# philip-bl/dctn

Measured on AMD Instinct MI355X. Metric: EPS-contraction windows/sec (fwd+bwd), higher is better.
Workload: dtype bf16; 1 GPU; cfg2 EPS[(3,4)]+linear bf16 B1024/GPU; parallelism=dp1

## Files before the change

dctn_amd/_lib.py:

```python
from __future__ import annotations

import ctypes
import os
import subprocess
from typing import Optional, Sequence

import torch

_HERE = os.path.dirname(os.path.abspath(__file__))
LIB_PATH = os.path.join(_HERE, "libdctn_amd.so")
CSRC = os.path.join(_HERE, "csrc")

F32, F64, BF16 = 0, 1, 2
PREC_EXACT, PREC_BF16, PREC_SPLIT, PREC_MASK = 0, 1, 2, 0xFF
OPT_F32_PREFER_HALVES, OPT_SMALL_CHUNKS, OPT_MAIN_KERNEL_ONLY, OPT_GENERIC_KERNELS = 1 << 8, 1 << 9, 1 << 10, 1 << 11
OPT_HEAD_FEATURES_BLOCKED4 = 1 << 12
ERR_BAD_SHAPE, ERR_BAD_DTYPE, ERR_UNSUPPORTED, ERR_WORKSPACE, ERR_LAUNCH, ERR_NULL = -1, -2, -3, -4, -5, -6
SAVED, PARTIAL = 1, 2
(EPS_FAMILY_GENERIC, EPS_FAMILY_Q2REG, EPS_FAMILY_BIGCORE_F32, EPS_FAMILY_HALVES, EPS_FAMILY_Q2REG_F32,
 EPS_FAMILY_BIGCORE_BF16X3) = range(6)
SBS_MATRIX_CORE_SWEEP = 1 << 8
SBS_WIDE_SWEEP = 1 << 9
BATCH_SRC_U8_TABLE, BATCH_SRC_ROWS = 0, 1
BATCH_IDENTITY_ORDER, BATCH_PAD_TAIL = 1, 2
# ... 16 lines not shown
    "dctn_device_limits": (c_int, [_IntP, _IntP]),
    "dctn_eps_family": (c_int, [c_int] * 9),
    "dctn_eps_fwd_workspace_bytes": (c_size, [c_int] * 7 + [c_int] * 2),
    "dctn_eps_fwd": (c_int, [c_void, _I64x5, c_void, c_void, c_void, c_size] + [c_int] * 7 + [c_int, c_int, c_void]),
    "dctn_eps_saved_bytes": (c_size, [c_int] * 7 + [c_int] * 2),
    "dctn_eps_fwd_save": (c_int, [c_void, _I64x5, c_void, c_void, c_void, c_size, c_void, c_size] + [c_int] * 7 + [c_int, c_int, c_void]),
    "dctn_eps_bwd_saved": (c_int, [c_void, _I64x5, c_void, c_void, c_void, c_size, c_void, c_void, c_void, c_size]
                           + [c_int] * 7 + [c_int, c_int, c_void]),
    "dctn_eps_fwd_stats_workspace_bytes": (c_size, [c_int] * 7 + [c_int] * 2),
    "dctn_eps_fwd_stats": (c_int, [c_void, _I64x5, c_void, c_void, c_void, c_size] + [c_int] * 7 + [c_int, c_int, c_void]),
    "dctn_eps_bwd_workspace_bytes": (c_size, [c_int] * 7 + [c_int] * 4),
    "dctn_eps_bwd": (c_int, [c_void, _I64x5, c_void, c_void, c_void, c_void, c_void, c_size]
                     + [c_int] * 7 + [c_int, c_int, c_void]),
    "dctn_eps_head_fwd": (c_int, [c_void, _I64x5, c_void, c_void, c_void, c_void, c_void] + [c_int] * 8 + [c_int, c_int, c_void]),
    "dctn_eps_head_bwd_workspace_bytes": (c_size, [c_int] * 8 + [c_int, c_int]),
    "dctn_eps_head_bwd": (c_int, [c_void, _I64x5, c_void, c_void, c_void, c_void, c_void, c_void, c_void, c_size]
                          + [c_int] * 8 + [c_int, c_int, c_void]),
    "dctn_ce_loss_fwd": (c_int, [c_void, c_void, c_void, c_i64, c_int, c_int, c_void]),
    "dctn_ce_loss_fwd_grad": (c_int, [c_void, c_void, c_void, c_void, c_i64, c_int, c_int, c_void]),
    "dctn_ce_loss_bwd": (c_int, [c_void, c_void, c_void, c_void, c_i64, c_int, c_int, c_void]),
    "dctn_sgd_l2_num_partials": (c_int, [c_i64]),
    "dctn_sgd_l2_step": (c_int, [c_void, c_void, c_void, c_void, c_i64, c_i64, ctypes.c_float, ctypes.c_float,
                                 ctypes.c_float, c_int, c_int, c_void]),
    "dctn_sgd_l2_step_master": (c_int, [c_void] * 5 + [c_i64, c_i64, ctypes.c_float, ctypes.c_float, ctypes.c_float,
                                        c_int, c_void]),
    "dctn_adam_state_bytes": (c_size, []),
    "dctn_adam_l2_num_partials": (c_int, [c_i64]),
    "dctn_adam_l2_step": (c_int, [c_void] * 6 + [c_i64, c_i64, ctypes.c_double, ctypes.c_double, ctypes.c_float,
                                  ctypes.c_float, ctypes.c_float, c_int, c_void]),
    "dctn_adam_l2_step_master": (c_int, [c_void] * 7 + [c_i64, c_i64, ctypes.c_double, ctypes.c_double, ctypes.c_float,
# ... 221 lines not shown
```

dctn_amd/csrc/capi.hip:

```cpp
#include "common.h"

#include <stdio.h>
#include <stdlib.h>

#include <algorithm>
#include <atomic>

static std::atomic<const char*> g_last_kernel{"none"};
void dctn_set_last_kernel(const char* name) { g_last_kernel.store(name, std::memory_order_relaxed); }

const DctnDev& dctn_dev() {
  static const DctnDev d = [] {
    DctnDev r{256, 160 * 1024};
    int dev = 0, v = 0;
    if (hipGetDevice(&dev) == hipSuccess) {
      if (hipDeviceGetAttribute(&v, hipDeviceAttributeMultiprocessorCount, dev) == hipSuccess && v > 0) r.cus = v;
      if (hipDeviceGetAttribute(&v, hipDeviceAttributeMaxSharedMemoryPerMultiprocessor, dev) == hipSuccess && v >= 64 * 1024) r.lds = v;
    }
    int cus = 0, lds = 0;
    const char* lim = getenv("DCTN_DEVICE_LIMITS");
    if (lim && sscanf(lim, "%d,%d", &cus, &lds) == 2) {
      if (cus > 0 && cus < r.cus) r.cus = cus;
      if (lds > 0 && lds < r.lds) r.lds = lds;
    }
// ... 144 lines not shown
                           int dtype, int policy) {
  if (!dtype_ok(dtype)) return DCTN_ERR_BAD_DTYPE;
  if (Cout < 1) return DCTN_ERR_BAD_SHAPE;
  const int blk = policy & DCTN_OPT_HEAD_FEATURES_BLOCKED4;
  const int rc = eps_fill_params(p, x_strides, C, B, H, W, Q, K, O, policy & ~blk);
  p.opts |= blk;
  return rc;
}

static bool eps_head_next(const EpsP& p, int rc) {
  return rc == DCTN_ERR_UNSUPPORTED && !(p.opts & DCTN_OPT_HEAD_FEATURES_BLOCKED4);
}

extern "C" {

int dctn_version(void) { return 507; }

const char* dctn_last_kernel(void) { return g_last_kernel.load(std::memory_order_relaxed); }

int dctn_device_limits(int* cus, int* lds_bytes) {
  if (!cus || !lds_bytes) return DCTN_ERR_NULL;
  *cus = dctn_dev().cus;
  *lds_bytes = dctn_dev().lds;
  return DCTN_OK;
}

const char* dctn_strerror(int code) {
  switch (code) {
    case DCTN_OK: return "ok";
    case DCTN_ERR_BAD_SHAPE: return "inconsistent shape";
    case DCTN_ERR_BAD_DTYPE: return "unknown dtype code";
// ... 119 lines not shown
  if (rc != DCTN_OK) return rc;
  const int precision = policy & DCTN_PREC_MASK;
  hipStream_t st = (hipStream_t)stream;
  rc = eps_head_fwd_mfma(x, core, head_weight, head_bias, features, logits, p, Cout, dtype, precision, st);
  if (!eps_head_next(p, rc)) return rc;
  return eps_head_fwd_q2f32(x, core, head_weight, head_bias, features, logits, p, Cout, dtype, precision, st);
}

size_t dctn_eps_head_bwd_workspace_bytes(int C, int B, int H, int W, int Q, int K, int O, int Cout, int dtype,
                                         int policy) {
  EpsP p;
  const int precision = policy & DCTN_PREC_MASK;
  if (!eps_query_params(p, C, B, H, W, Q, K, O, policy & ~DCTN_OPT_HEAD_FEATURES_BLOCKED4)) return 0;
  const size_t a = eps_head_bwd_mfma_workspace(p, Cout, dtype, precision), b = eps_head_bwd_q2f32_workspace(p, Cout, dtype, precision);
  return (a > b ? a : b) + 256;
}

int dctn_eps_head_bwd(const void* x, const int64_t x_strides[5], const void* features, const void* dLogits,
                      const void* head_weight, void* dCore, void* dWeight, void* dBias, void* workspace,
                      size_t workspace_bytes, int C, int B, int H, int W, int Q, int K, int O, int Cout,
                      int dtype, int policy, void* stream) {
  if (!x || !features || !dLogits || !head_weight || !dCore || !x_strides) return DCTN_ERR_NULL;
  EpsP p;
  int rc = eps_head_params(p, x_strides, C, B, H, W, Q, K, O, Cout, dtype, policy);
  if (rc != DCTN_OK) return rc;
  const int precision = policy & DCTN_PREC_MASK;
  hipStream_t st = (hipStream_t)stream;
  rc = eps_head_bwd_mfma(x, features, dLogits, head_weight, dCore, dWeight, dBias, workspace, workspace_bytes, p, Cout, dtype,
                         precision, st);
  if (!eps_head_next(p, rc)) return rc;
// ... 81 lines not shown
```

dctn_amd/csrc/common.h:

```cpp
#pragma once
#include <hip/hip_runtime.h>
#include <stdint.h>

#include "../../include/dctn_amd.h"

typedef __bf16 bf16_t;

template <typename S> struct AccOf { typedef float type; };
template <> struct AccOf<double> { typedef double type; };

#define DCTN_WAVE 64

#ifndef DCTN_WT_FEATURES
#define DCTN_WT_FEATURES 16
#endif
#ifndef DCTN_WT_TILES
#define DCTN_WT_TILES 0
#endif

struct DctnDev { int cus; int lds; };
const DctnDev& dctn_dev();
int dctn_lds_wg_max();
long long dctn_resident_wgs(size_t lds_bytes, int lo, int hi);
bool dctn_lds_optin(const void* fn, size_t bytes);
// ... 103 lines not shown
int eps_fwd_halves(const void* x, const void* core, void* out, void* ws, size_t ws_bytes, const EpsP& p, int dtype,
                   hipStream_t st, void* saved = nullptr);
size_t eps_bwd_halves_workspace(const EpsP& p, int dtype, int need_dx, int need_dcore);
int eps_bwd_halves(const void* x, const void* core, const void* dY, void* dX, void* dCore, void* ws, size_t ws_bytes,
                   const EpsP& p, int dtype, hipStream_t st, const void* saved = nullptr, size_t saved_bytes = 0);

int eps_fwd_mfma(const void* x, const void* core, void* out, const EpsP& p, int dtype,
                 int precision, hipStream_t st, double* stats = nullptr);
int eps_out_stats(const void* y, long long n, int dtype, double* stats, hipStream_t st);
size_t eps_bwd_mfma_workspace(const EpsP& p, int dtype, int precision, int need_dx, int need_dcore);
int eps_bwd_mfma(const void* x, const void* core, const void* dY, void* dX, void* dCore, void* ws,
                 size_t ws_bytes, const EpsP& p, int dtype, int precision, hipStream_t st);
int eps_head_fwd_mfma(const void* x, const void* core, const void* head_w, const void* bias, void* feat, void* logits,
                      const EpsP& p, int Cout, int dtype, int precision, hipStream_t st);
size_t eps_head_bwd_mfma_workspace(const EpsP& p, int Cout, int dtype, int precision);
int eps_head_bwd_mfma(const void* x, const void* feat, const void* dLogits, const void* head_w, void* dCore,
                      void* dW, void* dBias, void* ws, size_t ws_bytes, const EpsP& p, int Cout, int dtype,
                      int precision, hipStream_t st);

struct SbsShape {
  int n;
  const int *out_sizes, *bond_sizes, *pos_h, *pos_w;
  int C, B, H, W, q, dtype;
};
static inline SbsShape sbs_string(SbsShape many, int i) {
  many.out_sizes += i * many.n;
  many.bond_sizes += i * many.n;
  many.pos_h += i * many.n;
  many.pos_w += i * many.n;
  return many;
// ... 35 lines not shown
```

dctn_amd/csrc/eps_mfma.hip:

```cpp
#include "common.h"

#include <cstdlib>
#include <type_traits>

typedef __attribute__((ext_vector_type(8))) __bf16 bf16x8;
typedef __attribute__((ext_vector_type(16))) float f32x16;
typedef __attribute__((ext_vector_type(8))) float f32x8;
typedef __attribute__((ext_vector_type(2))) int int2v;
typedef __attribute__((ext_vector_type(4))) int int4v;
typedef __attribute__((ext_vector_type(2))) float f32x2;

namespace {

constexpr int ilog2(int v) { return v <= 1 ? 0 : 1 + ilog2(v >> 1); }

template <typename S> __device__ __forceinline__ float to_f32(S v) { return (float)v; }

__device__ __forceinline__ float half_sum(float v) {
  const int iv = __float_as_int(v);
  const int2v r = __builtin_amdgcn_permlane32_swap(iv, iv, false, false);
  return __int_as_float(r[0]) + __int_as_float(r[1]);
}

__device__ __forceinline__ void swap_halves(float& a, float& b) {
// ... 33 lines not shown
  const int g = lane >> 4, q = (lane >> 2) & 3, pp = lane & 3;
  const int lc = 2 * (g & 1) + (pp >> 1), half = pp & 1;
  const int row = 8 * (g >> 1) + q;
  t.rd_lo = row * LROW + (((lc + (row >> 1)) & 3) << 3) + 4 * half;
  t.rd_hi = (row + 4) * LROW + (((lc + ((row + 4) >> 1)) & 3) << 3) + 4 * half;
  return t;
}
__device__ __forceinline__ bf16x8 tr_frag(const short* tile, int ks, const TrLane& t) {
  typedef __attribute__((address_space(3))) s16x4 lds_s16x4;
  const s16x4 lo = __builtin_amdgcn_ds_read_tr16_b64_v4i16((lds_s16x4*)(tile + t.rd_lo + ks * 16 * LROW));
  const s16x4 hi = __builtin_amdgcn_ds_read_tr16_b64_v4i16((lds_s16x4*)(tile + t.rd_hi + ks * 16 * LROW));
  const s16x8 v = {lo[0], lo[1], lo[2], lo[3], hi[0], hi[1], hi[2], hi[3]};
  return __builtin_bit_cast(bf16x8, v);
}

struct FastDiv {
  unsigned M, s1, s2;
};
__device__ __forceinline__ unsigned fdiv(unsigned n, const FastDiv& d) {
  const unsigned t = __umulhi(d.M, n);
  return (t + ((n - t) >> d.s1)) >> d.s2;
}

#define MFMA_MAXN 16
struct MfmaP {
  int C, B, K, O, Ho, Wo;
  int P;
  int npg;
  int spc, nchunks;
  unsigned foffb[MFMA_MAXN];
  unsigned rowoffb[MFMA_MAXN];
  unsigned s1b, s2b, s3b, s4b;
  unsigned x_bytes;
  unsigned o_bytes, o_s1b;
  FastDiv div_wo;
  int rowvec_ok;
  int vec_ok;
  int Cout;
  unsigned hw_rowb, hw_bytes;
  int ncb;
  int skew;
  int opts;
#ifdef DCTN_STAMPS
  unsigned long long* stamps;
#endif
};

#ifdef DCTN_STAMPS
#define DCTN_STAMP(P, SLOT)                                                                      \
  do {                                                                                           \
    __builtin_amdgcn_sched_barrier(0);                                                           \
    unsigned long long t_;                                                                       \
    asm volatile("s_memrealtime %0\n\ts_waitcnt lgkmcnt(0)" : "=s"(t_)::"memory");               \
    if ((P).stamps && threadIdx.x == 0) (P).stamps[(long long)blockIdx.x * 8 + (SLOT)] = t_;     \
    __builtin_amdgcn_sched_barrier(0);                                                           \
  } while (0)
// ... 212 lines not shown
  } else {
#pragma unroll
    for (int o = 0; o < OP; ++o)
      if (o < O) {
        if constexpr (sizeof(S) == 2)
          __builtin_amdgcn_raw_buffer_store_b16((unsigned short)(pack_bf16(v[o], 0.f) & 0xffffu), rs, voff,
                                                soff + 2u * o, 0);
        else
          __builtin_amdgcn_raw_buffer_store_b32(__float_as_uint(v[o]), rs, voff, soff + 4u * o, 0);
      }
  }
}

struct WaveJob {
  int b0, b1;
  unsigned voff_x;
  unsigned voff_o;
  int pos;
  bool valid;
};
__device__ __forceinline__ WaveJob wave_job(const MfmaP& p, int waves_per_block, int esz, bool grouped = false) {
  const int nb = gridDim.x;
  const int vb = (nb % 8 == 0) ? (int)(blockIdx.x % 8) * (nb / 8) + (int)(blockIdx.x / 8) : (int)blockIdx.x;
  const int wave = __builtin_amdgcn_readfirstlane(vb * waves_per_block + (int)(threadIdx.x >> 6));
  int chunk = wave / p.npg, pg = wave - chunk * p.npg;
  if (grouped) {
    const int cb = vb / p.npg;
    pg = vb - cb * p.npg;
    chunk = __builtin_amdgcn_readfirstlane(cb * waves_per_block + (int)(threadIdx.x >> 6));
    if (cb >= p.ncb) chunk = p.nchunks;
  }
  WaveJob j;
  j.b0 = chunk < p.nchunks ? chunk * p.spc : 0;
  j.b1 = chunk < p.nchunks ? (j.b0 + p.spc < p.B ? j.b0 + p.spc : p.B) : 0;
  if (grouped && p.skew > 0) {
    const int w = __builtin_amdgcn_readfirstlane((int)(threadIdx.x >> 6)), half = waves_per_block / 2;
    const int n_old = p.spc + p.skew, n_young = p.spc - p.skew;
    const int s0 = (vb / p.npg) * waves_per_block * p.spc + (w < half ? w * n_old : half * n_old + (w - half) * n_young);
    const int s1 = s0 + (w < half ? n_old : n_young);
    const bool live = vb / p.npg < p.ncb && s0 < p.B;
    j.b0 = live ? s0 : 0;
    j.b1 = live ? (s1 < p.B ? s1 : p.B) : 0;
  }
  j.pos = pg * 64 + (int)(threadIdx.x & 63);
  j.valid = j.pos < p.P;
  const unsigned pu = j.valid ? (unsigned)j.pos : 0u;
  const unsigned ho = fdiv(pu, p.div_wo), wo = pu - ho * (unsigned)p.Wo;
  j.voff_x = j.valid ? ho * p.s2b + wo * p.s3b : p.x_bytes;
  j.voff_o = j.valid ? pu * (unsigned)(p.O * esz) : p.o_bytes;
  return j;
}

template <int N0>
__device__ __forceinline__ void build_p0(const float (*xv)[2], bf16x8 (&X)[(1 << N0) / 16],
                                         bf16x8 (&Y)[(1 << N0) / 16]) {
  constexpr int KS = (1 << N0) / 16;
  const f32x2 x1 = {xv[N0 - 1][0], xv[N0 - 1][1]}, x2 = {xv[N0 - 2][0], xv[N0 - 2][1]};
  const f32x2 m01 = bmul2(xv[N0 - 3][0], x2), m23 = bmul2(xv[N0 - 3][1], x2);
// ... 565 lines not shown
    if (tid < HEADT_GS * 16) {
      const int sl = tid >> 4, cc = tid & 15;
      if (sl < ng && cc < p.Cout) {
        float t = bias_s[cc];
#pragma unroll
        for (int w = 0; w < HEADT_WAVES; ++w) t += hsum[w][sl][cc];
        logits[(long long)(g0 + sl) * p.Cout + cc] = (bf16_t)t;
      }
    }
  }
  DCTN_STAMP(p, 6);
}

constexpr int BWD_WAVES = 8;
constexpr size_t dcore_dyn_lds_bytes(int mt) { return (size_t)BWD_WAVES * (1 + mt) * 64 * 32 * sizeof(short); }

__device__ __forceinline__ void head_dw_role_waves(const bf16_t* __restrict__ feat, const bf16_t* __restrict__ dL,
                                                   bf16_t* __restrict__ dW, int B, int Cout, long long F, int n_dw,
                                                   int rw, float* __restrict__ lds, const MfmaP& p);
template <typename S, int N0, int N1, int OP, bool XVEC, bool OVEC, int ROWS, int HEADC, int DWROLE = 0>
__global__ __launch_bounds__(64 * (BWD_WAVES + DWROLE)) void eps_bwd_dcore_q2reg_k(const S* __restrict__ x,
                                                             const S* __restrict__ dY,
                                                             const S* __restrict__ hw,
                                                             const S* __restrict__ feat,
                                                             float* __restrict__ partial,
                                                             float* __restrict__ dwpart, MfmaP p,
                                                             S* __restrict__ dW, int n_dw) {
  constexpr int N = N0 + N1, A = 1 << N0, BN = 1 << N1, KS = A / 16, MT = BN * OP / 32;
  constexpr int AT = A >= 32 ? A / 32 : 1;
  constexpr int LOGO = ilog2(OP);
  constexpr bool LDST = A == 32 && MT <= 2;
  __shared__ float red[BWD_WAVES][32 * 32];
  extern __shared__ __attribute__((aligned(16))) unsigned char dsm[];
  const int tid = threadIdx.x, lane = tid & 63, r = lane & 31, h = lane >> 5, wv = tid >> 6;
  DCTN_STAMP(p, 0);
  if constexpr (DWROLE > 0) {
    static_assert(HEADC > 0 && HEADC <= 16 && LDST && OVEC && XVEC && sizeof(S) == 2 && OP == 4, "the dW role rides the HEADMM path");
    const int rw = __builtin_amdgcn_readfirstlane(wv) - BWD_WAVES;
    if (rw >= 0) {
      head_dw_role_waves(feat, dY, dW, p.B, p.Cout, (long long)p.P * OP, n_dw, rw,
                         reinterpret_cast<float*>(dsm + dcore_dyn_lds_bytes(MT) + 8192), p);
      return;
    }
#ifdef DCTN_DWROLE_PRIO
    __builtin_amdgcn_s_setprio(DCTN_DWROLE_PRIO);
#endif
  }
  short* tiles = reinterpret_cast<short*>(dsm) + wv * ((1 + MT) * 64 * LROW);
  const TrLane trl = tr_lane(lane);

  bf16x8 ident[2];
#pragma unroll
  for (int sp = 0; sp < 2; ++sp)
#pragma unroll
    for (int j = 0; j < 8; ++j) ident[sp][j] = (bf16_t)((16 * sp + 8 * h + j == r) ? 1.f : 0.f);

  f32x16 acc[MT][AT];
#pragma unroll
  for (int t = 0; t < MT; ++t)
#pragma unroll
    for (int a = 0; a < AT; ++a)
#pragma unroll
      for (int v = 0; v < 16; ++v) acc[t][a][v] = 0.f;

  const WaveJob job = wave_job(p, BWD_WAVES, (int)sizeof(S), HEADC > 0);
  const __amdgpu_buffer_rsrc_t rs_x = make_rsrc(x, p.x_bytes);
  const __amdgpu_buffer_rsrc_t rs_dy = make_rsrc(HEADC > 0 ? feat : dY, p.o_bytes);
  constexpr bool HEADMM = HEADC > 0 && HEADC <= 16 && LDST && OVEC && XVEC && sizeof(S) == 2 && OP == 4;
  float hwf[HEADC > 0 && !HEADMM ? HEADC : 1][OP];
  float dwacc[HEADC > 0 && !HEADMM ? HEADC : 1][OP];
#pragma unroll
  for (int c = 0; c < (HEADC > 0 && !HEADMM ? HEADC : 1); ++c)
#pragma unroll
    for (int o = 0; o < OP; ++o) dwacc[c][o] = 0.f;
  constexpr int DLW = HEADC > 0 ? HEADC / 2 : 1;
  const unsigned* dl32 = reinterpret_cast<const unsigned*>(dY);
  unsigned dlraw[DLW];
  RawRow<S, OP> rr[HEADC > 0 && !HEADMM ? HEADC : 1];
  constexpr bool LATE = HEADC > 0 && LDST && !HEADMM;
  auto issue_head_weight = [&]() {
    if constexpr (HEADC > 0 && !HEADMM) {
      const __amdgpu_buffer_rsrc_t rs_hw = make_rsrc(hw, p.hw_bytes);
      const unsigned voff_hw = job.valid ? (unsigned)job.pos * (unsigned)(OP * 2) : p.hw_bytes;
// ... 52 lines not shown
    }
  };
  if constexpr (HEADMM) {
    static_assert(BWD_WAVES * 64 * 16 == 16 * 64 * OP * 2, "one 16-byte load per thread stages the weight slice");
    RawWindow<S, N, XVEC, ROWS> rawm;
    if (job.b0 < job.b1) issue_window<S, N, XVEC, ROWS>(rs_x, job.voff_x, (unsigned)job.b0 * p.s1b, p, rawm);
    const unsigned dl_bytes = (unsigned)p.B * (unsigned)p.Cout * 2u, dlrow = (unsigned)p.Cout * 2u;
    const __amdgpu_buffer_rsrc_t rs_dl = make_rsrc(dY, dl_bytes);
    const int slot = 4 * (r >> 3) + (r & 3);
    const bool rlow = ((r >> 2) & 1) == 0;
    u32x4 fa;
    auto issue_group = [&](int g0) {
      const unsigned voff_a = (r < 16 && g0 + slot < job.b1 && 8 * h < p.Cout) ? (unsigned)slot * dlrow + 16u * h : dl_bytes;
      fa = __builtin_amdgcn_raw_buffer_load_b128(rs_dl, voff_a, (unsigned)g0 * dlrow, 0);
    };
    u32x4 wv4;
    {
      const __amdgpu_buffer_rsrc_t rs_hw = make_rsrc(hw, p.hw_bytes);
      const int e = 2 * tid, c = e >> 6, posl = e & 63, pos = job.pos - lane + posl;
      const unsigned voff = pos < p.P ? (unsigned)pos * (unsigned)(OP * 2) : p.hw_bytes;
      wv4 = __builtin_amdgcn_raw_buffer_load_b128(rs_hw, voff, (unsigned)c * p.hw_rowb, 0);
      if (pos + 1 >= p.P) { wv4.z = 0u; wv4.w = 0u; }
    }
    issue_group(job.b0);
    *reinterpret_cast<u32x4*>(dsm + dcore_dyn_lds_bytes(MT) + (size_t)tid * 16) = wv4;
    __syncthreads();
    const unsigned* wlds = reinterpret_cast<const unsigned*>(dsm + dcore_dyn_lds_bytes(MT));
    DCTN_STAMP(p, 1);
    for (int g0 = job.b0; g0 < job.b1; g0 += 8) {
      if (g0 != job.b0) issue_group(g0);
      f32x8 dyg[OP];
      auto group_products = [&]() {
        int4v a0, a1;
#pragma unroll
        for (int d = 0; d < 4; ++d) {
          const bool dv = 8 * h + 2 * d < p.Cout;
          const int v = (int)(d == 0 ? fa.x : d == 1 ? fa.y : d == 2 ? fa.z : fa.w);
          a0[d] = (dv && rlow) ? v : 0;
          a1[d] = (dv && !rlow) ? v : 0;
        }
        int4v bw[OP][2];
#pragma unroll
// ... 639 lines not shown
  const long long esz = dtype == DCTN_BF16 ? 2 : 4;
  {
    long long ext = 0;
    const long long dims[5] = {p.C, p.B, p.H, p.W, p.Q};
    for (int i = 0; i < 5; ++i) {
      if (p.s[i] < 0) return false;
      ext += (dims[i] - 1) * p.s[i];
    }
    if ((ext + 1) * esz >= (1LL << 31)) return false;
    if (p.Wn * p.O * esz >= (1LL << 31)) return false;
  }
  const int op = next_pow2(p.O);
  return op >= 2 ? op <= 16 : true;
}

FastDiv make_fastdiv(unsigned d) {
  FastDiv f;
  if (d <= 1) {
    f.M = 0; f.s1 = 0; f.s2 = 0;
    return f;
  }
  unsigned l = 0;
  while ((1ull << l) < d) ++l;
  f.M = (unsigned)(((1ull << 32) * ((1ull << l) - d)) / d + 1);
  f.s1 = 1;
  f.s2 = l - 1;
  return f;
}

void fill_mp(MfmaP& m, const EpsP& p, const void* x, int dtype) {
  const long long esz = dtype == DCTN_BF16 ? 2 : 4;
  for (int n = 0; n < p.N && n < MFMA_MAXN; ++n) {
    const int pos = n / p.C, ch = n - pos * p.C;
    const int dh = pos / p.K, dw = pos - dh * p.K;
    m.foffb[n] = (unsigned)((ch * p.s[0] + dh * p.s[2] + dw * p.s[3]) * esz);
  }
  m.s1b = (unsigned)(p.s[1] * esz); m.s2b = (unsigned)(p.s[2] * esz);
  m.s3b = (unsigned)(p.s[3] * esz); m.s4b = (unsigned)(p.s[4] * esz);
  long long ext = 0;
  const long long dims[5] = {p.C, p.B, p.H, p.W, p.Q};
  for (int i = 0; i < 5; ++i) ext += (dims[i] - 1) * p.s[i];
  m.x_bytes = (unsigned)((ext + 1) * esz);
  const int rows = p.K * p.C;
  for (int rw = 0; rw < MFMA_MAXN; ++rw) m.rowoffb[rw] = 0;
// ... 1 lines not shown
    const int dh = rw / p.C, ch = rw - dh * p.C;
    m.rowoffb[rw] = (unsigned)((ch * p.s[0] + dh * p.s[2]) * esz);
  }
  m.rowvec_ok = dtype == DCTN_BF16 && p.s[4] == 1 && p.s[3] == 2 && p.K <= 4 && rows <= MFMA_MAXN / 2 &&
                ((p.N == 9 && rows == 3) || (p.N == 8 && rows == 4));
  m.div_wo = make_fastdiv((unsigned)p.Wo);
  m.C = p.C; m.B = p.B; m.K = p.K; m.O = p.O; m.Ho = p.Ho; m.Wo = p.Wo;
  m.P = p.Ho * p.Wo;
  m.npg = (m.P + 63) / 64;
  m.spc = 1; m.nchunks = p.B;
  m.o_s1b = (unsigned)((long long)m.P * p.O * esz);
  m.o_bytes = (unsigned)(p.Wn * p.O * esz);
  m.vec_ok = p.s[4] == 1 && p.s[0] % 2 == 0 && p.s[1] % 2 == 0 && p.s[2] % 2 == 0 &&
             p.s[3] % 2 == 0 && ((uintptr_t)x % 4) == 0;
  m.Cout = 0; m.hw_rowb = 0; m.hw_bytes = 0; m.ncb = 0; m.skew = 0;
  m.opts = p.opts;
#ifdef DCTN_STAMPS
  m.stamps = g_stamps;
#endif
}

constexpr int FWD_BLOCKS_PER_CU = 4;

template <int N0, int N1, int OP>
constexpr size_t dcore_dyn_lds() {
  constexpr int A = 1 << N0, MT = (1 << N1) * OP / 32;
  return (A == 32 && MT <= 2) ? (size_t)BWD_WAVES * (1 + MT) * 64 * LROW * sizeof(short) : 0;
}
#define DCTN_DCORE_LAUNCH(KERNEL, G, B, DYN, ST, ...)                                                  \
  do {                                                                                                 \
// ... 68 lines not shown
                       (const S*)x, (const S*)dY, (const S*)nullptr, (const S*)nullptr, (float*)ws, (float*)nullptr, m, (S*)nullptr, 0);
  DCTN_CHECK_LAUNCH();
  if (m.opts & DCTN_OPT_MAIN_KERNEL_ONLY) return DCTN_PARTIAL;
  hipLaunchKernelGGL((eps_bwd_dcore_reduce_k<S>), dim3(BN * OP * AT), dim3(256), 0, st,
                     (const float*)ws, (S*)dCore, grid, A, BN, m.O, OP, AT * 32);
  DCTN_CHECK_LAUNCH();
  dctn_set_last_kernel("eps_bwd_mfma_q2reg");
  return DCTN_OK;
}

#ifndef DCTN_DCORE_SKEW
#define DCTN_DCORE_SKEW(spc) ((spc) / 3)
#endif

int plan_grouped(MfmaP& m) {
  if (m.npg > dctn_dev().cus) return 0;
  long long ncb = dctn_dev().cus / m.npg;
  const long long need = (m.B + BWD_WAVES - 1) / BWD_WAVES;
  if (ncb > need) ncb = need;
  m.spc = (int)((m.B + ncb * BWD_WAVES - 1) / (ncb * BWD_WAVES));
  m.nchunks = (m.B + m.spc - 1) / m.spc;
  m.ncb = (m.nchunks + BWD_WAVES - 1) / BWD_WAVES;
  long long blocks = (long long)m.ncb * m.npg;
  if (blocks >= 8) blocks = (blocks + 7) / 8 * 8;
  return blocks <= dctn_dev().cus ? (int)blocks : 0;
}

size_t head_dw_partial_bytes(const EpsP& p, int Cout) {
  const long long P = (long long)p.Ho * p.Wo, npg = (P + 63) / 64;
  if (npg > dctn_dev().cus) return 0;
  return (size_t)(dctn_dev().cus / npg) * ((size_t)Cout * (size_t)(P * p.O) + 16) * sizeof(float);
}

long long blocked4_bytes(const MfmaP& m) { return (long long)(m.B + 3) / 4 * 4 * m.P * m.O * 2; }
template <int N0, int N1, int OP>
bool head_blocked4_ok(const MfmaP& m) {
  constexpr int A = 1 << N0, MT = (1 << N1) * OP / 32;
  const long long F = (long long)m.P * OP;
  return A == 32 && MT <= 2 && OP == 4 && m.vec_ok && blocked4_bytes(m) < (1LL << 31) && !(m.opts & DCTN_OPT_SMALL_CHUNKS) &&
         F % 8 == 0 && F <= (long long)HEADT_WAVES * HEADT_MAXKS * 32;
}

template <int N0, int N1, int OP>
int bwd_head_launch_t(const void* x, const void* dL, const void* hw, const void* feat, void* dCore, void* dW,
                      void* dBias, void* ws, size_t core_ws_bytes, const MfmaP& m_in, hipStream_t st) {
  typedef bf16_t S;
  constexpr int A = 1 << N0, BN = 1 << N1, AT = A >= 32 ? A / 32 : 1;
  constexpr size_t DYN = dcore_dyn_lds<N0, N1, OP>();
  MfmaP m = m_in;
  const bool blk = (m.opts & DCTN_OPT_HEAD_FEATURES_BLOCKED4) != 0;
  if (m.O != OP || m.Cout < 2 || m.Cout > 16 || m.Cout % 2 != 0) return DCTN_ERR_UNSUPPORTED;
  if (((uintptr_t)dL % 4) != 0 || ((uintptr_t)hw % 4) != 0 || ((uintptr_t)feat % (blk ? 16 : 4)) != 0) return DCTN_ERR_UNSUPPORTED;
  if (blk && !head_blocked4_ok<N0, N1, OP>(m)) return DCTN_ERR_UNSUPPORTED;
  const int grid = plan_grouped(m);
  if (grid == 0) return DCTN_ERR_UNSUPPORTED;
  float* dwpart = reinterpret_cast<float*>(static_cast<unsigned char*>(ws) + core_ws_bytes);
  const long long nW = (long long)m.Cout * m.P * OP;
  constexpr int MT = BN * OP / 32;
  const bool headmm = A == 32 && MT <= 2 && OP == 4 && m.vec_ok;
  if (headmm && (long long)m.B * m.P * OP * 2 >= (1LL << 31)) return DCTN_ERR_UNSUPPORTED;
  const bool gemm = headmm;
  m.skew = headmm ? DCTN_DCORE_SKEW(m.spc) : 0;
  if (m.skew >= m.spc) m.skew = m.spc - 1;

  const dim3 g(grid), b(64 * BWD_WAVES);
  constexpr int NN = N0 + N1;
  constexpr int RW = NN == 9 ? 3 : 4;
  const int n_slices = (int)(((long long)m.P * OP + DWG_BFW - 1) / DWG_BFW);
  bool dwrole = false;
  if constexpr (A == 32 && MT <= 2 && OP == 4) {
    constexpr size_t RDYN = DYN + 8192 + DWR_LDS_BYTES;
#define DCTN_HEAD_ROLE_LAUNCH(ROWSV, HC)                                                                          \
  do {                                                                                                            \
    const void* kfn = (const void*)eps_bwd_dcore_q2reg_k<S, N0, N1, OP, true, true, ROWSV, HC, DWR_WAVES>;        \
    if (dctn_lds_optin(kfn, RDYN)) {                                                                              \
      hipLaunchKernelGGL((eps_bwd_dcore_q2reg_k<S, N0, N1, OP, true, true, ROWSV, HC, DWR_WAVES>), g,             \
                         dim3(64 * (BWD_WAVES + DWR_WAVES)), RDYN, st, (const S*)x, (const S*)dL, (const S*)hw,   \
                         (const S*)feat, (float*)ws, dwpart, m, (S*)dW, dW ? n_slices : 0);                       \
      dwrole = true;                                                                                              \
    }                                                                                                             \
  } while (0)
    if (blk && headmm) {
      if (m.rowvec_ok) {
        if (m.Cout <= 10) DCTN_HEAD_ROLE_LAUNCH(RW, 10); else DCTN_HEAD_ROLE_LAUNCH(RW, 16);
      } else {
        if (m.Cout <= 10) DCTN_HEAD_ROLE_LAUNCH(0, 10); else DCTN_HEAD_ROLE_LAUNCH(0, 16);
      }
    }
#undef DCTN_HEAD_ROLE_LAUNCH
  }
#define DCTN_HEAD_LAUNCH(XV, ROWSV, HC)                                                                        \
  DCTN_DCORE_LAUNCH((eps_bwd_dcore_q2reg_k<S, N0, N1, OP, XV, true, ROWSV, HC>), g, b, (DYN > 0 ? DYN + 8192 : 0), st, (const S*)x, \
                     (const S*)dL, (const S*)hw, (const S*)feat, (float*)ws, dwpart, m, (S*)nullptr, 0)
  if (dwrole) {
  } else if (m.rowvec_ok && m.vec_ok) {
    if (m.Cout <= 10) DCTN_HEAD_LAUNCH(true, RW, 10); else DCTN_HEAD_LAUNCH(true, RW, 16);
  } else if (m.vec_ok) {
    if (m.Cout <= 10) DCTN_HEAD_LAUNCH(true, 0, 10); else DCTN_HEAD_LAUNCH(true, 0, 16);
  } else {
    if (m.Cout <= 10) DCTN_HEAD_LAUNCH(false, 0, 10); else DCTN_HEAD_LAUNCH(false, 0, 16);
  }
#undef DCTN_HEAD_LAUNCH
  DCTN_CHECK_LAUNCH();
  if (m.opts & DCTN_OPT_MAIN_KERNEL_ONLY) return DCTN_PARTIAL;
  const int fw = blk ? DWG_BFW : DWG_FW;
  const int n_core = BN * OP * AT;
  if (dwrole) {
// ... 139 lines not shown
  const size_t core_ws = (eps_bwd_mfma_workspace(p, dtype, precision, 0, 1) + 255) / 256 * 256;
  MfmaP m;
  fill_mp(m, p, x, dtype);
  m.Cout = Cout;
  const long long rowb = (long long)m.P * p.O * 2;
  m.hw_rowb = (unsigned)rowb;
  m.hw_bytes = (unsigned)(rowb * Cout);
  if (p.N == 9) {
    if (p.O == 2) return bwd_head_launch_t<5, 4, 2>(x, dLogits, head_w, feat, dCore, dW, dBias, ws, core_ws, m, st);
    return bwd_head_launch_t<5, 4, 4>(x, dLogits, head_w, feat, dCore, dW, dBias, ws, core_ws, m, st);
  }
  if (p.O == 2) return bwd_head_launch_t<4, 4, 2>(x, dLogits, head_w, feat, dCore, dW, dBias, ws, core_ws, m, st);
  return bwd_head_launch_t<4, 4, 4>(x, dLogits, head_w, feat, dCore, dW, dBias, ws, core_ws, m, st);
}

int eps_head_fwd_mfma(const void* x, const void* core, const void* head_w, const void* bias, void* feat, void* logits,
                      const EpsP& p, int Cout, int dtype, int precision, hipStream_t st) {
  if (!head_family_ok(p, Cout, dtype, precision)) return DCTN_ERR_UNSUPPORTED;
  MfmaP m;
  fill_mp(m, p, x, dtype);
  m.Cout = Cout;
  const long long rowb = (long long)m.P * p.O * 2;
  m.hw_rowb = (unsigned)rowb;
  m.hw_bytes = (unsigned)(rowb * Cout);
  if (p.N == 9) {
    if (p.O == 2) return fwd_head_launch_t<5, 4, 2>(x, core, head_w, bias, feat, logits, m, st);
    return fwd_head_launch_t<5, 4, 4>(x, core, head_w, bias, feat, logits, m, st);
  }
  if (p.O == 2) return fwd_head_launch_t<4, 4, 2>(x, core, head_w, bias, feat, logits, m, st);
  return fwd_head_launch_t<4, 4, 4>(x, core, head_w, bias, feat, logits, m, st);
// ... 4 lines not shown
```

include/dctn_amd.h:

```cpp
#ifndef DCTN_AMD_H
#define DCTN_AMD_H

#include <stddef.h>
#include <stdint.h>

#ifdef __cplusplus
extern "C" {
#endif

enum { DCTN_F32 = 0, DCTN_F64 = 1, DCTN_BF16 = 2, DCTN_DTYPE_MASK = 0xFF };
enum { DCTN_SBS_MATRIX_CORE_SWEEP = 1 << 8 };
enum { DCTN_SBS_WIDE_SWEEP = 1 << 9 };

enum {
  DCTN_OK = 0,
  DCTN_ERR_BAD_SHAPE = -1,
  DCTN_ERR_BAD_DTYPE = -2,
  DCTN_ERR_UNSUPPORTED = -3,
  DCTN_ERR_WORKSPACE = -4,
  DCTN_ERR_LAUNCH = -5,
  DCTN_ERR_NULL = -6
};
enum {
  DCTN_SAVED = 1,
// ... 55 lines not shown
                      int C, int B, int H, int W, int Q, int K, int O,
                      int dtype, int policy, void* stream);
int dctn_eps_bwd_saved(const void* x, const int64_t x_strides[5], const void* core, const void* dY,
                       const void* saved, size_t saved_bytes,
                       void* dX, void* dCore, void* workspace, size_t workspace_bytes,
                       int C, int B, int H, int W, int Q, int K, int O,
                       int dtype, int policy, void* stream);

int dctn_eps_head_fwd(const void* x, const int64_t x_strides[5], const void* core, const void* head_weight,
                      const void* head_bias, void* features, void* logits,
                      int C, int B, int H, int W, int Q, int K, int O, int Cout,
                      int dtype, int policy, void* stream);

size_t dctn_eps_head_bwd_workspace_bytes(int C, int B, int H, int W, int Q, int K, int O, int Cout,
                                         int dtype, int policy);
int dctn_eps_head_bwd(const void* x, const int64_t x_strides[5], const void* features,
                      const void* dLogits, const void* head_weight, void* dCore, void* dWeight,
                      void* dBias, void* workspace, size_t workspace_bytes,
                      int C, int B, int H, int W, int Q, int K, int O, int Cout,
                      int dtype, int policy, void* stream);

size_t dctn_convsbs_workspace_bytes(int n_cores, const int* out_sizes, const int* bond_sizes,
                                    int C, int B, int H, int W, int q,
                                    const int* pos_h, const int* pos_w, int dtype, int backward);
int dctn_convsbs_fwd(const void* x, const int64_t x_strides[5], const void* const* cores,
                     void* out, int n_cores, const int* out_sizes, const int* bond_sizes,
                     const int* pos_h, const int* pos_w,
                     int C, int B, int H, int W, int q,
                     void* workspace, size_t workspace_bytes, int dtype, void* stream);
int dctn_convsbs_bwd(const void* x, const int64_t x_strides[5], const void* const* cores,
// ... 156 lines not shown
```

Before: 28.24 billion windows/s.

## Flatten dCore head-backward work split across position groups and batch segments

Adds a flat work distribution for the head-backward dCore kernel. The (position-group × batch) item space is split evenly over up to one workgroup per CU, and a wave may straddle two position groups, so two head-weight slices are loaded into LDS. The goal is to remove the load imbalance of the grouped plan when npg does not divide the CU count well. It costs extra LDS, a second slice load and more index arithmetic per wave, and it adds a plan-query API for inspection.

```diff
diff --git a/dctn_amd/_lib.py b/dctn_amd/_lib.py
--- a/dctn_amd/_lib.py
+++ b/dctn_amd/_lib.py
@@ -54,6 +54,7 @@
                      + [c_int] * 7 + [c_int, c_int, c_void]),
     "dctn_eps_head_fwd": (c_int, [c_void, _I64x5, c_void, c_void, c_void, c_void, c_void] + [c_int] * 8 + [c_int, c_int, c_void]),
     "dctn_eps_head_bwd_workspace_bytes": (c_size, [c_int] * 8 + [c_int, c_int]),
+    "dctn_eps_head_bwd_plan": (c_int, [c_int] * 8 + [c_int, c_int, c_int] + [_IntP] * 4),
     "dctn_eps_head_bwd": (c_int, [c_void, _I64x5, c_void, c_void, c_void, c_void, c_void, c_void, c_void, c_size]
                           + [c_int] * 8 + [c_int, c_int, c_void]),
     "dctn_ce_loss_fwd": (c_int, [c_void, c_void, c_void, c_i64, c_int, c_int, c_void]),
diff --git a/dctn_amd/csrc/capi.hip b/dctn_amd/csrc/capi.hip
--- a/dctn_amd/csrc/capi.hip
+++ b/dctn_amd/csrc/capi.hip
@@ -182,7 +182,7 @@
 
 extern "C" {
 
-int dctn_version(void) { return 507; }
+int dctn_version(void) { return 508; }
 
 const char* dctn_last_kernel(void) { return g_last_kernel.load(std::memory_order_relaxed); }
 
@@ -332,6 +332,15 @@
   if (!eps_query_params(p, C, B, H, W, Q, K, O, policy & ~DCTN_OPT_HEAD_FEATURES_BLOCKED4)) return 0;
   const size_t a = eps_head_bwd_mfma_workspace(p, Cout, dtype, precision), b = eps_head_bwd_q2f32_workspace(p, Cout, dtype, precision);
   return (a > b ? a : b) + 256;
+}
+
+int dctn_eps_head_bwd_plan(int C, int B, int H, int W, int Q, int K, int O, int Cout, int dtype, int policy, int workgroup,
+                           int* grid, int* flat, int* two_segment_waves, int* waves) {
+  if (!grid || !flat || !two_segment_waves || !waves) return DCTN_ERR_NULL;
+  if (!dtype_ok(dtype)) return DCTN_ERR_BAD_DTYPE;
+  EpsP p;
+  if (!eps_query_params(p, C, B, H, W, Q, K, O, policy & ~DCTN_OPT_HEAD_FEATURES_BLOCKED4) || Cout < 1) return DCTN_ERR_BAD_SHAPE;
+  return eps_head_bwd_mfma_plan(p, Cout, dtype, policy & DCTN_PREC_MASK, workgroup, grid, flat, two_segment_waves, waves);
 }
 
 int dctn_eps_head_bwd(const void* x, const int64_t x_strides[5], const void* features, const void* dLogits,
diff --git a/dctn_amd/csrc/common.h b/dctn_amd/csrc/common.h
--- a/dctn_amd/csrc/common.h
+++ b/dctn_amd/csrc/common.h
@@ -141,6 +141,8 @@
 int eps_head_fwd_mfma(const void* x, const void* core, const void* head_w, const void* bias, void* feat, void* logits,
                       const EpsP& p, int Cout, int dtype, int precision, hipStream_t st);
 size_t eps_head_bwd_mfma_workspace(const EpsP& p, int Cout, int dtype, int precision);
+int eps_head_bwd_mfma_plan(const EpsP& p, int Cout, int dtype, int precision, int workgroup, int* grid, int* flat,
+                           int* two_segment_waves, int* waves);
 int eps_head_bwd_mfma(const void* x, const void* feat, const void* dLogits, const void* head_w, void* dCore,
                       void* dW, void* dBias, void* ws, size_t ws_bytes, const EpsP& p, int Cout, int dtype,
                       int precision, hipStream_t st);
diff --git a/dctn_amd/csrc/dcore_plan.h b/dctn_amd/csrc/dcore_plan.h
--- /dev/null
+++ b/dctn_amd/csrc/dcore_plan.h
@@ -0,0 +1,170 @@
+#pragma once
+
+#if defined(__HIPCC__)
+#define DCP_HD __host__ __device__ __forceinline__
+#else
+#define DCP_HD inline
+#endif
+
+struct FastDiv {
+  unsigned M, s1, s2;
+};
+DCP_HD unsigned fdiv(unsigned n, const FastDiv& d) {
+#if defined(__HIP_DEVICE_COMPILE__)
+  const unsigned t = __umulhi(d.M, n);
+#else
+  const unsigned t = (unsigned)(((unsigned long long)d.M * n) >> 32);
+#endif
+  return (t + ((n - t) >> d.s1)) >> d.s2;
+}
+inline FastDiv make_fastdiv(unsigned d) {
+  FastDiv f;
+  if (d <= 1) {
+    f.M = 0; f.s1 = 0; f.s2 = 0;
+    return f;
+  }
+  unsigned l = 0;
+  while ((1ull << l) < d) ++l;
+  f.M = (unsigned)(((1ull << 32) * ((1ull << l) - d)) / d + 1);
+  f.s1 = 1;
+  f.s2 = l - 1;
+  return f;
+}
+
+#ifndef DCTN_DCORE_FLAT
+#define DCTN_DCORE_FLAT 1
+#endif
+#ifndef DCTN_DCORE_FLAT_YOUNG
+#define DCTN_DCORE_FLAT_YOUNG(q) (((q) + 1) / 3)
+#endif
+
+constexpr int DCORE_WAVES = 8;
+
+struct DcoreGrouped {
+  int spc, nchunks, ncb;
+  int grid;
+};
+inline DcoreGrouped dcore_grouped_plan(int B, int npg, int cus) {
+  DcoreGrouped g{1, B, 0, 0};
+  if (npg > cus) return g;
+  long long ncb = cus / npg;
+  const long long need = ((long long)B + DCORE_WAVES - 1) / DCORE_WAVES;
+  if (ncb > need) ncb = need;
+  g.spc = (int)((B + ncb * DCORE_WAVES - 1) / (ncb * DCORE_WAVES));
+  g.nchunks = (B + g.spc - 1) / g.spc;
+  g.ncb = (g.nchunks + DCORE_WAVES - 1) / DCORE_WAVES;
+  long long blocks = (long long)g.ncb * npg;
+  if (blocks >= 8) blocks = (blocks + 7) / 8 * 8;
+  g.grid = blocks <= cus ? (int)blocks : 0;
+  return g;
+}
+DCP_HD void dcore_grouped_wave(int B, int spc, int nchunks, int ncb, int skew, int cb, int w, int& b0, int& b1) {
+  int chunk = cb * DCORE_WAVES + w;
+  if (cb >= ncb) chunk = nchunks;
+  b0 = chunk < nchunks ? chunk * spc : 0;
+  b1 = chunk < nchunks ? (b0 + spc < B ? b0 + spc : B) : 0;
+  if (skew > 0) {
+    const int half = DCORE_WAVES / 2;
+    const int n_old = spc + skew, n_young = spc - skew;
+    const int s0 = cb * DCORE_WAVES * spc + (w < half ? w * n_old : half * n_old + (w - half) * n_young);
+    const int s1 = s0 + (w < half ? n_old : n_young);
+    const bool live = cb < ncb && s0 < B;
+    b0 = live ? s0 : 0;
+    b1 = live ? (s1 < B ? s1 : B) : 0;
+  }
+}
+DCP_HD int dcore_virtual_block(int blk, int grid) { return grid % 8 == 0 ? (blk % 8) * (grid / 8) + blk / 8 : blk; }
+
+struct DcoreFlat {
+  int G;
+  int ns;
+  int n0, r0;
+  int seg_lo;
+  FastDiv div_g, div_lo, div_hi;
+};
+struct DcoreWave {
+  int pg, b0, b1;
+  int pg_a, pg_b;
+  int items;
+};
+
+DCP_HD int dcore_seg_start(const DcoreFlat& f, int B, int e) {
+  const long long t = (long long)e * B;
+  return (int)(f.ns == 8 ? t >> 3 : t);
+}
+
+DCP_HD DcoreWave dcore_flat_wave(const DcoreFlat& f, int B, int npg, int blk, int w) {
+  const int v = dcore_virtual_block(blk, f.G);
+  const unsigned i0 = (unsigned)v * (unsigned)f.n0 + fdiv((unsigned)v * (unsigned)f.r0, f.div_g);
+  const unsigned i1 = (unsigned)(v + 1) * (unsigned)f.n0 + fdiv((unsigned)(v + 1) * (unsigned)f.r0, f.div_g);
+  const int n = (int)(i1 - i0);
+  int e = f.ns == 8 ? blk % 8 : 0;
+  int s_e = dcore_seg_start(f, B, e), s_e1 = dcore_seg_start(f, B, e + 1);
+  while (e + 1 < f.ns && i0 >= (unsigned)npg * (unsigned)s_e1) {
+    ++e;
+    s_e = s_e1;
+    s_e1 = dcore_seg_start(f, B, e + 1);
+  }
+  const int len = s_e1 - s_e;
+  const unsigned u = i0 - (unsigned)npg * (unsigned)s_e;
+  const int pg_a = (int)fdiv(u, len == f.seg_lo ? f.div_lo : f.div_hi);
+  const int sa = (int)u - pg_a * len;
+  const int na = n < len - sa ? n : len - sa;
+  int pg_b = pg_a + 1, sb = s_e;
+  if (pg_b == npg) {
+    pg_b = 0;
+    sb = s_e1;
+  }
+  const int s = w & 3, base = n >> 2, rem = n & 3;
+  const bool young = w >= 4;
+  const int q = base + (s < rem ? 1 : 0), c = s * base + (s < rem ? s : rem);
+  int k0, k1;
+  if (na > c && na < c + q) {
+    const int t = na - c;
+    const bool older_first = 2 * t >= q;
+    const bool second = young == older_first;
+    k0 = second ? c + t : c;
+    k1 = second ? c + q : c + t;
+  } else {
+    const int ny = DCTN_DCORE_FLAT_YOUNG(q), no = q - ny;
+    k0 = young ? c + no : c;
+    k1 = young ? c + q : c + no;
+  }
+  DcoreWave d;
+  const bool in_a = k1 <= na;
+  d.pg = in_a ? pg_a : pg_b;
+  d.b0 = in_a ? s_e + sa + k0 : sb + (k0 - na);
+  d.b1 = in_a ? s_e + sa + k1 : sb + (k1 - na);
+  d.pg_a = pg_a;
+  d.pg_b = (na < n && pg_b != pg_a) ? pg_b : -1;
+  d.items = n;
+  return d;
+}
+
+inline DcoreFlat dcore_flat_plan(int B, int npg, int cus, const DcoreGrouped& g, int skew) {
+  DcoreFlat f{};
+  const long long T = (long long)npg * B;
+  if (!DCTN_DCORE_FLAT || g.grid == 0 || T >= (1LL << 31)) return f;
+  long long G = (T + DCORE_WAVES - 1) / DCORE_WAVES;
+  if (G > cus) G = cus;
+  const long long n_max = (T + G - 1) / G;
+  int old_max = 0;
+  for (int s = 0; s < DCORE_WAVES / 2; ++s) {
+    int a0, a1, c0, c1;
+    dcore_grouped_wave(B, g.spc, g.nchunks, g.ncb, skew, 0, s, a0, a1);
+    dcore_grouped_wave(B, g.spc, g.nchunks, g.ncb, skew, 0, s + DCORE_WAVES / 2, c0, c1);
+    if ((a1 - a0) + (c1 - c0) > old_max) old_max = (a1 - a0) + (c1 - c0);
+  }
+  if ((n_max + 3) / 4 >= old_max) return f;
+  int ns = (G % 8 == 0 && B / 8 >= 1 && B / 8 >= n_max - 1) ? 8 : 1;
+  if (ns == 1 && B < n_max - 1) return f;
+  f.G = (int)G;
+  f.ns = ns;
+  f.n0 = (int)(T / G);
+  f.r0 = (int)(T % G);
+  f.seg_lo = B / ns;
+  f.div_g = make_fastdiv((unsigned)G);
+  f.div_lo = make_fastdiv((unsigned)f.seg_lo);
+  f.div_hi = make_fastdiv((unsigned)f.seg_lo + 1);
+  return f;
+}
diff --git a/dctn_amd/csrc/eps_mfma.hip b/dctn_amd/csrc/eps_mfma.hip
--- a/dctn_amd/csrc/eps_mfma.hip
+++ b/dctn_amd/csrc/eps_mfma.hip
@@ -1,4 +1,5 @@
 #include "common.h"
+#include "dcore_plan.h"
 
 #include <cstdlib>
 #include <type_traits>
@@ -71,13 +72,6 @@
   return __builtin_bit_cast(bf16x8, v);
 }
 
-struct FastDiv {
-  unsigned M, s1, s2;
-};
-__device__ __forceinline__ unsigned fdiv(unsigned n, const FastDiv& d) {
-  const unsigned t = __umulhi(d.M, n);
-  return (t + ((n - t) >> d.s1)) >> d.s2;
-}
 
 #define MFMA_MAXN 16
 struct MfmaP {
@@ -97,6 +91,7 @@
   unsigned hw_rowb, hw_bytes;
   int ncb;
   int skew;
+  DcoreFlat flat;
   int opts;
 #ifdef DCTN_STAMPS
   unsigned long long* stamps;
@@ -339,11 +334,14 @@
 
 struct WaveJob {
   int b0, b1;
+  int pg;
+  int pg_a, pg_b;
   unsigned voff_x;
   unsigned voff_o;
   int pos;
   bool valid;
 };
+template <bool FLAT = false>
 __device__ __forceinline__ WaveJob wave_job(const MfmaP& p, int waves_per_block, int esz, bool grouped = false) {
   const int nb = gridDim.x;
   const int vb = (nb % 8 == 0) ? (int)(blockIdx.x % 8) * (nb / 8) + (int)(blockIdx.x / 8) : (int)blockIdx.x;
@@ -359,14 +357,23 @@
   j.b0 = chunk < p.nchunks ? chunk * p.spc : 0;
   j.b1 = chunk < p.nchunks ? (j.b0 + p.spc < p.B ? j.b0 + p.spc : p.B) : 0;
   if (grouped && p.skew > 0) {
-    const int w = __builtin_amdgcn_readfirstlane((int)(threadIdx.x >> 6)), half = waves_per_block / 2;
-    const int n_old = p.spc + p.skew, n_young = p.spc - p.skew;
-    const int s0 = (vb / p.npg) * waves_per_block * p.spc + (w < half ? w * n_old : half * n_old + (w - half) * n_young);
-    const int s1 = s0 + (w < half ? n_old : n_young);
-    const bool live = vb / p.npg < p.ncb && s0 < p.B;
-    j.b0 = live ? s0 : 0;
-    j.b1 = live ? (s1 < p.B ? s1 : p.B) : 0;
-  }
+    const int w = __builtin_amdgcn_readfirstlane((int)(threadIdx.x >> 6));
+    dcore_grouped_wave(p.B, p.spc, p.nchunks, p.ncb, p.skew, vb / p.npg, w, j.b0, j.b1);
+  }
+  j.pg_a = pg;
+  j.pg_b = -1;
+  if constexpr (FLAT) {
+    if (p.flat.G > 0) {
+      const int w = __builtin_amdgcn_readfirstlane((int)(threadIdx.x >> 6));
+      const DcoreWave d = dcore_flat_wave(p.flat, p.B, p.npg, (int)blockIdx.x, w);
+      pg = __builtin_amdgcn_readfirstlane(d.pg);
+      j.b0 = __builtin_amdgcn_readfirstlane(d.b0);
+      j.b1 = __builtin_amdgcn_readfirstlane(d.b1);
+      j.pg_a = __builtin_amdgcn_readfirstlane(d.pg_a);
+      j.pg_b = __builtin_amdgcn_readfirstlane(d.pg_b);
+    }
+  }
+  j.pg = pg;
   j.pos = pg * 64 + (int)(threadIdx.x & 63);
   j.valid = j.pos < p.P;
   const unsigned pu = j.valid ? (unsigned)j.pos : 0u;
@@ -962,6 +969,8 @@
 
 constexpr int BWD_WAVES = 8;
 constexpr size_t dcore_dyn_lds_bytes(int mt) { return (size_t)BWD_WAVES * (1 + mt) * 64 * 32 * sizeof(short); }
+constexpr size_t DCORE_HW_SLICE_BYTES = 8192, DCORE_HW_LDS_BYTES = 2 * DCORE_HW_SLICE_BYTES;
+static_assert(BWD_WAVES == DCORE_WAVES, "dcore_plan.h plans the waves of this kernel");
 
 __device__ __forceinline__ void head_dw_role_waves(const bf16_t* __restrict__ feat, const bf16_t* __restrict__ dL,
                                                    bf16_t* __restrict__ dW, int B, int Cout, long long F, int n_dw,
@@ -987,7 +996,7 @@
     const int rw = __builtin_amdgcn_readfirstlane(wv) - BWD_WAVES;
     if (rw >= 0) {
       head_dw_role_waves(feat, dY, dW, p.B, p.Cout, (long long)p.P * OP, n_dw, rw,
-                         reinterpret_cast<float*>(dsm + dcore_dyn_lds_bytes(MT) + 8192), p);
+                         reinterpret_cast<float*>(dsm + dcore_dyn_lds_bytes(MT) + DCORE_HW_LDS_BYTES), p);
       return;
     }
 #ifdef DCTN_DWROLE_PRIO
@@ -1011,10 +1020,10 @@
 #pragma unroll
       for (int v = 0; v < 16; ++v) acc[t][a][v] = 0.f;
 
-  const WaveJob job = wave_job(p, BWD_WAVES, (int)sizeof(S), HEADC > 0);
+  constexpr bool HEADMM = HEADC > 0 && HEADC <= 16 && LDST && OVEC && XVEC && sizeof(S) == 2 && OP == 4;
+  const WaveJob job = wave_job<HEADMM>(p, BWD_WAVES, (int)sizeof(S), HEADC > 0);
   const __amdgpu_buffer_rsrc_t rs_x = make_rsrc(x, p.x_bytes);
   const __amdgpu_buffer_rsrc_t rs_dy = make_rsrc(HEADC > 0 ? feat : dY, p.o_bytes);
-  constexpr bool HEADMM = HEADC > 0 && HEADC <= 16 && LDST && OVEC && XVEC && sizeof(S) == 2 && OP == 4;
   float hwf[HEADC > 0 && !HEADMM ? HEADC : 1][OP];
   float dwacc[HEADC > 0 && !HEADMM ? HEADC : 1][OP];
 #pragma unroll
@@ -1097,18 +1106,25 @@
       const unsigned voff_a = (r < 16 && g0 + slot < job.b1 && 8 * h < p.Cout) ? (unsigned)slot * dlrow + 16u * h : dl_bytes;
       fa = __builtin_amdgcn_raw_buffer_load_b128(rs_dl, voff_a, (unsigned)g0 * dlrow, 0);
     };
-    u32x4 wv4;
-    {
-      const __amdgpu_buffer_rsrc_t rs_hw = make_rsrc(hw, p.hw_bytes);
-      const int e = 2 * tid, c = e >> 6, posl = e & 63, pos = job.pos - lane + posl;
+    static_assert(BWD_WAVES * 64 * 16 == DCORE_HW_SLICE_BYTES, "a slice is one 16-byte load per thread");
+    const __amdgpu_buffer_rsrc_t rs_hw = make_rsrc(hw, p.hw_bytes);
+    auto load_slice = [&](int pg) {
+      const int e = 2 * tid, c = e >> 6, posl = e & 63, pos = pg * 64 + posl;
       const unsigned voff = pos < p.P ? (unsigned)pos * (unsigned)(OP * 2) : p.hw_bytes;
-      wv4 = __builtin_amdgcn_raw_buffer_load_b128(rs_hw, voff, (unsigned)c * p.hw_rowb, 0);
-      if (pos + 1 >= p.P) { wv4.z = 0u; wv4.w = 0u; }
-    }
+      u32x4 v = __builtin_amdgcn_raw_buffer_load_b128(rs_hw, voff, (unsigned)c * p.hw_rowb, 0);
+      if (pos + 1 >= p.P) { v.z = 0u; v.w = 0u; }
+      return v;
+    };
+    const u32x4 wv4 = load_slice(job.pg_a);
+    const bool two_slices = job.pg_b >= 0;
+    u32x4 wv4b = u32x4{0u, 0u, 0u, 0u};
+    if (two_slices) wv4b = load_slice(job.pg_b);
     issue_group(job.b0);
     *reinterpret_cast<u32x4*>(dsm + dcore_dyn_lds_bytes(MT) + (size_t)tid * 16) = wv4;
+    if (two_slices) *reinterpret_cast<u32x4*>(dsm + dcore_dyn_lds_bytes(MT) + DCORE_HW_SLICE_BYTES + (size_t)tid * 16) = wv4b;
     __syncthreads();
-    const unsigned* wlds = reinterpret_cast<const unsigned*>(dsm + dcore_dyn_lds_bytes(MT));
+    const unsigned* wlds = reinterpret_cast<const unsigned*>(dsm + dcore_dyn_lds_bytes(MT) +
+                                                              (job.pg == job.pg_a ? 0 : DCORE_HW_SLICE_BYTES));
     DCTN_STAMP(p, 1);
     for (int g0 = job.b0; g0 < job.b1; g0 += 8) {
       if (g0 != job.b0) issue_group(g0);
@@ -1778,20 +1794,6 @@
   return op >= 2 ? op <= 16 : true;
 }
 
-FastDiv make_fastdiv(unsigned d) {
-  FastDiv f;
-  if (d <= 1) {
-    f.M = 0; f.s1 = 0; f.s2 = 0;
-    return f;
-  }
-  unsigned l = 0;
-  while ((1ull << l) < d) ++l;
-  f.M = (unsigned)(((1ull << 32) * ((1ull << l) - d)) / d + 1);
-  f.s1 = 1;
-  f.s2 = l - 1;
-  return f;
-}
-
 void fill_mp(MfmaP& m, const EpsP& p, const void* x, int dtype) {
   const long long esz = dtype == DCTN_BF16 ? 2 : 4;
   for (int n = 0; n < p.N && n < MFMA_MAXN; ++n) {
@@ -1823,6 +1825,7 @@
   m.vec_ok = p.s[4] == 1 && p.s[0] % 2 == 0 && p.s[1] % 2 == 0 && p.s[2] % 2 == 0 &&
              p.s[3] % 2 == 0 && ((uintptr_t)x % 4) == 0;
   m.Cout = 0; m.hw_rowb = 0; m.hw_bytes = 0; m.ncb = 0; m.skew = 0;
+  m.flat = DcoreFlat{};
   m.opts = p.opts;
 #ifdef DCTN_STAMPS
   m.stamps = g_stamps;
@@ -1921,16 +1924,24 @@
 #endif
 
 int plan_grouped(MfmaP& m) {
-  if (m.npg > dctn_dev().cus) return 0;
-  long long ncb = dctn_dev().cus / m.npg;
-  const long long need = (m.B + BWD_WAVES - 1) / BWD_WAVES;
-  if (ncb > need) ncb = need;
-  m.spc = (int)((m.B + ncb * BWD_WAVES - 1) / (ncb * BWD_WAVES));
-  m.nchunks = (m.B + m.spc - 1) / m.spc;
-  m.ncb = (m.nchunks + BWD_WAVES - 1) / BWD_WAVES;
-  long long blocks = (long long)m.ncb * m.npg;
-  if (blocks >= 8) blocks = (blocks + 7) / 8 * 8;
-  return blocks <= dctn_dev().cus ? (int)blocks : 0;
+  const DcoreGrouped g = dcore_grouped_plan(m.B, m.npg, dctn_dev().cus);
+  if (g.grid == 0) return 0;
+  m.spc = g.spc;
+  m.nchunks = g.nchunks;
+  m.ncb = g.ncb;
+  return g.grid;
+}
+int plan_head_dcore(MfmaP& m, bool headmm) {
+  int grid = plan_grouped(m);
+  if (grid == 0) return 0;
+  m.skew = headmm ? DCTN_DCORE_SKEW(m.spc) : 0;
+  if (m.skew >= m.spc) m.skew = m.spc - 1;
+  m.flat = DcoreFlat{};
+  if (headmm) {
+    m.flat = dcore_flat_plan(m.B, m.npg, dctn_dev().cus, DcoreGrouped{m.spc, m.nchunks, m.ncb, grid}, m.skew);
+    if (m.flat.G > 0) grid = m.flat.G;
+  }
+  return grid;
 }
 
 size_t head_dw_partial_bytes(const EpsP& p, int Cout) {
@@ -1959,16 +1970,14 @@
   if (m.O != OP || m.Cout < 2 || m.Cout > 16 || m.Cout % 2 != 0) return DCTN_ERR_UNSUPPORTED;
   if (((uintptr_t)dL % 4) != 0 || ((uintptr_t)hw % 4) != 0 || ((uintptr_t)feat % (blk ? 16 : 4)) != 0) return DCTN_ERR_UNSUPPORTED;
   if (blk && !head_blocked4_ok<N0, N1, OP>(m)) return DCTN_ERR_UNSUPPORTED;
-  const int grid = plan_grouped(m);
+  constexpr int MT = BN * OP / 32;
+  const bool headmm = A == 32 && MT <= 2 && OP == 4 && m.vec_ok;
+  const int grid = plan_head_dcore(m, headmm);
   if (grid == 0) return DCTN_ERR_UNSUPPORTED;
   float* dwpart = reinterpret_cast<float*>(static_cast<unsigned char*>(ws) + core_ws_bytes);
   const long long nW = (long long)m.Cout * m.P * OP;
-  constexpr int MT = BN * OP / 32;
-  const bool headmm = A == 32 && MT <= 2 && OP == 4 && m.vec_ok;
   if (headmm && (long long)m.B * m.P * OP * 2 >= (1LL << 31)) return DCTN_ERR_UNSUPPORTED;
   const bool gemm = headmm;
-  m.skew = headmm ? DCTN_DCORE_SKEW(m.spc) : 0;
-  if (m.skew >= m.spc) m.skew = m.spc - 1;
 
   const dim3 g(grid), b(64 * BWD_WAVES);
   constexpr int NN = N0 + N1;
@@ -1976,7 +1985,7 @@
   const int n_slices = (int)(((long long)m.P * OP + DWG_BFW - 1) / DWG_BFW);
   bool dwrole = false;
   if constexpr (A == 32 && MT <= 2 && OP == 4) {
-    constexpr size_t RDYN = DYN + 8192 + DWR_LDS_BYTES;
+    constexpr size_t RDYN = DYN + DCORE_HW_LDS_BYTES + DWR_LDS_BYTES;
 #define DCTN_HEAD_ROLE_LAUNCH(ROWSV, HC)                                                                          \
   do {                                                                                                            \
     const void* kfn = (const void*)eps_bwd_dcore_q2reg_k<S, N0, N1, OP, true, true, ROWSV, HC, DWR_WAVES>;        \
@@ -1997,7 +2006,7 @@
 #undef DCTN_HEAD_ROLE_LAUNCH
   }
 #define DCTN_HEAD_LAUNCH(XV, ROWSV, HC)                                                                        \
-  DCTN_DCORE_LAUNCH((eps_bwd_dcore_q2reg_k<S, N0, N1, OP, XV, true, ROWSV, HC>), g, b, (DYN > 0 ? DYN + 8192 : 0), st, (const S*)x, \
+  DCTN_DCORE_LAUNCH((eps_bwd_dcore_q2reg_k<S, N0, N1, OP, XV, true, ROWSV, HC>), g, b, (DYN > 0 ? DYN + DCORE_HW_LDS_BYTES : 0), st, (const S*)x, \
                      (const S*)dL, (const S*)hw, (const S*)feat, (float*)ws, dwpart, m, (S*)nullptr, 0)
   if (dwrole) {
   } else if (m.rowvec_ok && m.vec_ok) {
@@ -2167,6 +2176,34 @@
   return bwd_head_launch_t<4, 4, 4>(x, dLogits, head_w, feat, dCore, dW, dBias, ws, core_ws, m, st);
 }
 
+int eps_head_bwd_mfma_plan(const EpsP& p, int Cout, int dtype, int precision, int workgroup, int* grid, int* flat,
+                           int* two_segment_waves, int* waves) {
+  if (!head_family_ok(p, Cout, dtype, precision)) return DCTN_ERR_UNSUPPORTED;
+  MfmaP m{};
+  m.B = p.B;
+  m.P = p.Ho * p.Wo;
+  m.npg = (m.P + 63) / 64;
+  const int A = 1 << (p.N == 9 ? 5 : 4), MT = 16 * p.O / 32;
+  const int g = plan_head_dcore(m, A == 32 && MT <= 2 && p.O == 4);
+  if (g == 0) return DCTN_ERR_UNSUPPORTED;
+  if (workgroup < 0 || workgroup >= g) return DCTN_ERR_BAD_SHAPE;
+  *grid = g;
+  *flat = m.flat.G > 0;
+  *two_segment_waves = 0;
+  for (int w = 0; w < DCORE_WAVES; ++w) {
+    int* o = waves + 3 * w;
+    if (m.flat.G > 0) {
+      const DcoreWave d = dcore_flat_wave(m.flat, m.B, m.npg, workgroup, w);
+      o[0] = d.pg; o[1] = d.b0; o[2] = d.b1;
+    } else {
+      const int vb = dcore_virtual_block(workgroup, g), cb = vb / m.npg;
+      o[0] = vb - cb * m.npg;
+      dcore_grouped_wave(m.B, m.spc, m.nchunks, m.ncb, m.skew, cb, w, o[1], o[2]);
+    }
+  }
+  return DCTN_OK;
+}
+
 int eps_head_fwd_mfma(const void* x, const void* core, const void* head_w, const void* bias, void* feat, void* logits,
                       const EpsP& p, int Cout, int dtype, int precision, hipStream_t st) {
   if (!head_family_ok(p, Cout, dtype, precision)) return DCTN_ERR_UNSUPPORTED;
diff --git a/include/dctn_amd.h b/include/dctn_amd.h
--- a/include/dctn_amd.h
+++ b/include/dctn_amd.h
@@ -93,6 +93,8 @@
 
 size_t dctn_eps_head_bwd_workspace_bytes(int C, int B, int H, int W, int Q, int K, int O, int Cout,
                                          int dtype, int policy);
+int dctn_eps_head_bwd_plan(int C, int B, int H, int W, int Q, int K, int O, int Cout, int dtype, int policy,
+                           int workgroup, int* grid, int* flat, int* two_segment_waves, int* waves);
 int dctn_eps_head_bwd(const void* x, const int64_t x_strides[5], const void* features,
                       const void* dLogits, const void* head_weight, void* dCore, void* dWeight,
                       void* dBias, void* workspace, size_t workspace_bytes,
```

Result: slower. 26.92 billion windows/s (-4.7%).
